# EugenHotaj/pytorch-generative

Measured on NVIDIA H100. Metric: images/sec training step (ImageGPT CIFAR-10 32x32), higher is better.
Workload: dtype bf16

## Files before the change

### pytorch_generative_b200/csrc/pg_gemm.cu

```cuda
#include <stdlib.h>
#include <string.h>

#include "../../include/pg_b200.h"
#include "pg_common.cuh"

namespace {

constexpr int BM = 128;
constexpr int BK = 64;
constexpr int A_STAGE_BYTES = BM * BK * 2;
constexpr int SMEM_LIMIT = 232448;

constexpr int MAX_CONV_TAPS = 225;
struct ConvGeom {
  int mode, H, W, C, T;
  int cslabs;
  int nbpt;
  int8_t dy[MAX_CONV_TAPS], dx[MAX_CONV_TAPS];
};

struct GemmParams {
  ConvGeom conv;
  int M, N, K;
  int num_m_blk, num_n_blk;
  int k_iters;
  int k_per_split;
  int splits;
  int stages;
  int epi_tma, epi_nbuf, epi_buf_bytes, epi_in_bytes;
  int off_old, off_res0, off_res1, off_aux, off_f32, off_pre, off_bf16;
  int epi_smem;
  int store_deriv;
  int res_bf16;
  float* a_rowsum;
  float* split_part;
  float* rowsum_part;
  pg_gemm_epilogue epi;
};

struct EpiMaps {
  CUtensorMap res0, res1, aux, out_f32, out_pre, out_bf16;
  CUtensorMap bias;
};

template <bool BWD, int ACT, int N>
__device__ __forceinline__ void act_as(float (&x)[N]) {
#pragma unroll
  for (int i = 0; i < N; ++i) x[i] = BWD ? pg_act_bwd(ACT, x[i]) : pg_act_fwd(ACT, x[i]);
}
template <bool BWD, int N>
__device__ __forceinline__ void act_n(int act, float (&x)[N]) {
  switch (act) {
    case PG_ACT_RELU: act_as<BWD, PG_ACT_RELU>(x); break;
    case PG_ACT_GELU: act_as<BWD, PG_ACT_GELU>(x); break;
    case PG_ACT_ELU: act_as<BWD, PG_ACT_ELU>(x); break;
    case PG_ACT_TANH: act_as<BWD, PG_ACT_TANH>(x); break;
    case PG_ACT_GIVEN: act_as<BWD, PG_ACT_GIVEN>(x); break;
    case PG_ACT_RELU_OUT: act_as<BWD, PG_ACT_RELU_OUT>(x); break;
    case PG_ACT_ELU_OUT: act_as<BWD, PG_ACT_ELU_OUT>(x); break;
    default: act_as<BWD, PG_ACT_NONE>(x); break;
  }
}

__device__ __forceinline__ void epilogue_row32(const GemmParams& p, int row, int col0, int ncols, bool first_split,
                                               const uint32_t (&acc)[32], float* out_f32, int64_t ld_out_f32,
                                               bool accumulate) {
  const pg_gemm_epilogue& e = p.epi;
  float v[32];
#pragma unroll
  for (int i = 0; i < 32; ++i) v[i] = __uint_as_float(acc[i]) * e.alpha;

  if (first_split && e.bias) {
    for (int i = 0; i < ncols; ++i) v[i] += __ldg(e.bias + col0 + i);
  }
  if (e.dact != PG_ACT_NONE) {
    const bf16* aux = reinterpret_cast<const bf16*>(e.aux) + (size_t)row * e.ld_aux + col0;
    for (int i = 0; i < ncols; ++i) v[i] *= pg_act_bwd(e.dact, __bfloat162float(aux[i]));
  }
#pragma unroll
  for (int which = 0; which < 2; ++which) {
    const float* rp = which == 0 ? e.res0 : e.res1;
    if (first_split && rp && p.res_bf16) {
      const bf16* r = reinterpret_cast<const bf16*>(rp) + (size_t)row * e.ld_res + col0;
      for (int i = 0; i < ncols; ++i) v[i] += __bfloat162float(r[i]);
    } else if (first_split && rp) {
      const float* r = rp + (size_t)row * e.ld_res + col0;
      for (int i = 0; i < ncols; ++i) v[i] += r[i];
    }
  }
  if (out_f32) {
    float* o = out_f32 + (size_t)row * ld_out_f32 + col0;
    if (accumulate) {
      for (int i = 0; i < ncols; ++i) o[i] += v[i];
    } else {
      for (int i = 0; i < ncols; ++i) o[i] = v[i];
    }
  }
  if (e.out_pre) {
    bf16* o = reinterpret_cast<bf16*>(e.out_pre) + (size_t)row * e.ld_out_pre + col0;
    float d[32];
#pragma unroll
    for (int i = 0; i < 32; ++i) d[i] = v[i];
    if (p.store_deriv) act_n<true>(e.act, d);
    for (int i = 0; i < ncols; ++i) o[i] = __float2bfloat16(d[i]);
  }
  if (e.out_bf16) {
    bf16* o = reinterpret_cast<bf16*>(e.out_bf16) + (size_t)row * e.ld_out_bf16 + col0;
    if (e.act != PG_ACT_NONE) act_n<false>(e.act, v);
    for (int i = 0; i < ncols; ++i) o[i] = __float2bfloat16(v[i]);
  }
}

constexpr int GEMM_THREADS = 384;
constexpr int XP_LD = 68;
constexpr int XP_BYTES = 64 * XP_LD * 4;
constexpr int MAX_STAGES = 8;
constexpr int MAX_EPI_BUFS = 4;
constexpr int EPI_F32_BYTES = 16 * 32 * 4;
constexpr int EPI_BF16_BYTES = 16 * 32 * 2;
constexpr int EPI_BIAS_BYTES = 128 * 4;
constexpr int PRODUCER_REGS = 56;
constexpr int CONSUMER_REGS = 224;
constexpr uint32_t XPOSE_BAR = 1;
constexpr uint32_t ROWSUM_BAR = 3;
constexpr uint32_t MMA_TURN_BAR = 4;

struct WorkItem {
  int m_blk, n_blk, ks, k0, k1;
};
__device__ __forceinline__ WorkItem work_item(const GemmParams& p, int tile) {
  WorkItem w;
  w.n_blk = tile % p.num_n_blk;
  const int rest = tile / p.num_n_blk;
  w.m_blk = rest % p.num_m_blk;
  w.ks = rest / p.num_m_blk;
  w.k0 = w.ks * p.k_per_split;
  w.k1 = min(w.k0 + p.k_per_split, p.k_iters);
  return w;
}

template <int BN, bool A_MN, bool B_MN>
__device__ __forceinline__ void consumer_mainloop(uint8_t* smem, uint64_t* full_bar, uint64_t* empty_bar, int stages,
                                                  const WorkItem& w, int& s, uint32_t& ph, float (&acc)[2][BN / 2],
                                                  int turn_bar) {
  constexpr int STAGE_BYTES = A_STAGE_BYTES + BN * BK * 2;
  const int lane = threadIdx.x & 31;
  int prev = -1;
  for (int kit = w.k0; kit < w.k1; ++kit) {
    mbar_wait(&full_bar[s], ph);
    const uint32_t a_addr = smem_u32(smem + s * STAGE_BYTES);
    const uint32_t b_addr = smem_u32(smem + s * STAGE_BYTES) + A_STAGE_BYTES;
    const uint64_t b_base = B_MN ? wgmma_desc_sw128(b_addr, BK * 128, 1024) : wgmma_desc_sw128(b_addr, 16, 1024);
    wgmma_fence();
#pragma unroll
    for (int kk = 0; kk < BK / 16; ++kk) {
#pragma unroll
      for (int sl = 0; sl < 2; ++sl) {
        const uint32_t sa = a_addr + sl * (64 * 128);
        const uint64_t a_base = A_MN ? wgmma_desc_sw128(sa, BK * 128, 1024) : wgmma_desc_sw128(sa, 16, 1024);
        Wgmma<BN>::template ss<A_MN ? 1 : 0, B_MN ? 1 : 0>(acc[sl], a_base + (uint64_t)(A_MN ? kk * 128 : kk * 2),
                                                         b_base + (uint64_t)(B_MN ? kk * 128 : kk * 2),
                                                         (kit > w.k0 || kk > 0) ? 1u : 0u);
      }
    }
    wgmma_commit();
    wgmma_wait<1>();
    if (prev >= 0) {
      __syncwarp();
      if (lane == 0) mbar_arrive(&empty_bar[prev]);
    }
    prev = s;
    if (++s == stages) { s = 0; ph ^= 1; }
  }
  if (turn_bar >= 0) named_bar_arrive((uint32_t)turn_bar, 256);
  wgmma_wait<0>();
#pragma unroll
  for (int sl = 0; sl < 2; ++sl) wgmma_hold(acc[sl]);
  if (prev >= 0) {
    __syncwarp();
    if (lane == 0) mbar_arrive(&empty_bar[prev]);
  }
}

template <int BN>
__device__ __forceinline__ void consumer_epilogue(const GemmParams& p, const WorkItem& w, const float (&acc)[2][BN / 2],
                                                  float* xp, uint32_t xbar) {
  constexpr int CSTEPS = (BN + 63) / 64;
  const int t = threadIdx.x & 127, lane = threadIdx.x & 31, wi = (threadIdx.x >> 5) & 3;
  const int r = t & 63, half = t >> 6;
#pragma unroll 1
  for (int step = 0; step < 2 * CSTEPS; ++step) {
    const int sl = step / CSTEPS, c0 = (step - sl * CSTEPS) * 64;
    const int row = w.m_blk * BM + sl * 64 + r;
    named_bar_sync(xbar, 128);
#pragma unroll
    for (int q = 0; q < 2; ++q) {
#pragma unroll
      for (int j = 0; j < BN / 8; ++j) {
        if (q == sl && j * 8 >= c0 && j * 8 < c0 + 64) {
          const int col = j * 8 - c0 + 2 * (lane & 3), fr = wi * 16 + (lane >> 2);
          *reinterpret_cast<float2*>(xp + fr * XP_LD + col) = make_float2(acc[q][4 * j], acc[q][4 * j + 1]);
          *reinterpret_cast<float2*>(xp + (fr + 8) * XP_LD + col) = make_float2(acc[q][4 * j + 2], acc[q][4 * j + 3]);
        }
      }
    }
    named_bar_sync(xbar, 128);
    const int col0 = w.n_blk * BN + c0 + half * 32;
    if (c0 + half * 32 < BN && row < p.M && col0 < p.N) {
      uint32_t v[32];
#pragma unroll
      for (int u = 0; u < 8; ++u) {
        const float4 x = *reinterpret_cast<const float4*>(xp + r * XP_LD + half * 32 + 4 * u);
        v[4 * u] = __float_as_uint(x.x); v[4 * u + 1] = __float_as_uint(x.y);
        v[4 * u + 2] = __float_as_uint(x.z); v[4 * u + 3] = __float_as_uint(x.w);
      }
      const bool split = p.split_part != nullptr;
      epilogue_row32(p, row, col0, min(32, p.N - col0), w.ks == 0, v,
                     split ? p.split_part + (size_t)w.ks * p.M * p.N : p.epi.out_f32,
                     split ? (int64_t)p.N : p.epi.ld_out_f32, !split && p.epi.accumulate);
    }
  }
}

struct EpiRing {
  uint8_t* buf;
  float* bias;
  uint64_t* in_bar;
  uint64_t* bias_bar;
};
__device__ __forceinline__ EpiRing epi_ring(const GemmParams& p, uint8_t* epi, int cw) {
  const int wq = cw * 4 + ((threadIdx.x >> 5) & 3);
  EpiRing r;
  r.buf = epi + wq * p.epi_nbuf * p.epi_buf_bytes;
  r.bias = reinterpret_cast<float*>(epi + 8 * p.epi_nbuf * p.epi_buf_bytes + cw * EPI_BIAS_BYTES);
  r.in_bar = reinterpret_cast<uint64_t*>(epi + p.epi_smem) + 2 * MAX_STAGES + wq * MAX_EPI_BUFS;
  r.bias_bar = reinterpret_cast<uint64_t*>(epi + p.epi_smem) + 2 * MAX_STAGES + 8 * MAX_EPI_BUFS + cw;
  return r;
}

constexpr int EK_GENERIC = 0;
constexpr int EK_BIAS = 1, EK_GIVEN = 2, EK_RES0 = 4, EK_RES1 = 8, EK_F32 = 16, EK_BF16 = 32, EK_GELU2 = 64;
constexpr int EK_PLAIN = EK_BF16;
constexpr int EK_BIAS_BF16 = EK_BIAS | EK_BF16;
constexpr int EK_BIAS_GELU2 = EK_BIAS | EK_GELU2;
constexpr int EK_GIVEN_BF16 = EK_GIVEN | EK_BF16;
constexpr int EK_BIAS_RES_F32 = EK_BIAS | EK_RES0 | EK_F32;
constexpr int EK_BIAS_RES2_F32 = EK_BIAS | EK_RES0 | EK_RES1 | EK_F32;

__device__ __forceinline__ bool subtile_live(const GemmParams& p, int row, int col) { return row < p.M && col < p.N; }

template <int BN>
__device__ __forceinline__ void epi_load(const GemmParams& p, const EpiMaps& tm, const WorkItem& w, const EpiRing& r,
                                         int g0, int j) {
  constexpr int CG = BN / 32;
  const int wi = (threadIdx.x >> 5) & 3;
  const int b = (g0 + j) % p.epi_nbuf;
  uint8_t* buf = r.buf + b * p.epi_buf_bytes;
  const int col = w.n_blk * BN + (j % CG) * 32, row = w.m_blk * BM + (j / CG) * 64 + wi * 16;
  if (!subtile_live(p, row, col)) {
    mbar_arrive(&r.in_bar[b]);
    return;
  }
  mbar_arrive_expect_tx(&r.in_bar[b], (uint32_t)p.epi_in_bytes);
  if (p.off_old >= 0) tma_load_3d(buf + p.off_old, &tm.out_f32, &r.in_bar[b], col, row, 0);
  if (p.off_res0 >= 0) tma_load_2d(buf + p.off_res0, &tm.res0, &r.in_bar[b], col, row);
  if (p.off_res1 >= 0) tma_load_2d(buf + p.off_res1, &tm.res1, &r.in_bar[b], col, row);
  if (p.off_aux >= 0) tma_load_2d(buf + p.off_aux, &tm.aux, &r.in_bar[b], col, row);
}

template <int BN>
__device__ __forceinline__ void epi_prologue(const GemmParams& p, const EpiMaps& tm, const WorkItem& w, const EpiRing& r,
                                             int item) {
  if ((threadIdx.x & 31) != 0 || !p.epi_in_bytes) return;
  bulk_wait_group_read<1>();
  for (int j = 0; j < p.epi_nbuf - 1 && j < 2 * (BN / 32); ++j) epi_load<BN>(p, tm, w, r, item * 2 * (BN / 32), j);
}

template <int BN>
__device__ __forceinline__ void epi_bias(const GemmParams& p, const EpiMaps& tm, const WorkItem& w, const EpiRing& r) {
  if ((threadIdx.x & 127) != 0 || !p.epi.bias) return;
  mbar_arrive_expect_tx(r.bias_bar, BN * 4);
  tma_load_1d(r.bias, &tm.bias, r.bias_bar, w.n_blk * BN);
}

template <int BN, int EK, bool ACT>
__device__ __forceinline__ void consumer_epilogue_tma(const GemmParams& p, const EpiMaps& tm, const WorkItem& w,
                                                      const float (&acc)[2][BN / 2], const EpiRing& r, int item) {
  constexpr int CG = BN / 32, NSUB = 2 * CG;
  constexpr bool G = EK == EK_GENERIC;
  const pg_gemm_epilogue& e = p.epi;
  const int lane = threadIdx.x & 31, wi = (threadIdx.x >> 5) & 3;
  const int nb = p.epi_nbuf, g0 = item * NSUB;
  const bool bias = G ? e.bias != nullptr : (EK & EK_BIAS) != 0;
  const bool has_in = G ? p.epi_in_bytes != 0 : (EK & (EK_GIVEN | EK_RES0)) != 0;
  const bool f32_out = G ? p.off_f32 >= 0 : (EK & EK_F32) != 0;
  const bool bf16_out = G ? p.off_bf16 >= 0 : (EK & (EK_BF16 | EK_GELU2)) != 0;
  const bool pre_out = G ? p.off_pre >= 0 : (EK & EK_GELU2) != 0;
  if (bias) mbar_wait(r.bias_bar, (uint32_t)item & 1u);
  const uint32_t rb = lane >> 2;
  const uint32_t f32_base = rb * 128 + ((((uint32_t)lane >> 1) & 1u) ^ (rb & 7u)) * 16 + (lane & 1) * 8;
  const uint32_t bf_base = rb * 64 + ((rb >> 1) & 3u) * 16 + (lane & 3) * 4;
  auto f32_at = [&](int jj, int hi) { return (f32_base ^ (uint32_t)(jj << 5)) + hi * 1024; };
  auto bf_at = [&](int jj, int hi) { return (bf_base ^ (uint32_t)(jj << 4)) + hi * 512; };
  int b = g0 % nb;
  uint32_t par = (uint32_t)(g0 / nb) & 1u;
#pragma unroll(G ? 1 : NSUB)
  for (int i = 0; i < NSUB; ++i) {
    const int sl = i / CG, cg = i - sl * CG;
    uint8_t* buf = r.buf + b * p.epi_buf_bytes;
    float v[16];
#pragma unroll
    for (int q = 0; q < 2; ++q)
#pragma unroll
      for (int c = 0; c < CG; ++c)
        if (q == sl && c == cg) {
#pragma unroll
          for (int k = 0; k < 16; ++k) v[k] = acc[q][c * 16 + k];
        }
    if (has_in) mbar_wait(&r.in_bar[b], par);
    if (G) {
#pragma unroll
      for (int k = 0; k < 16; ++k) v[k] *= e.alpha;
    }
    if (bias) {
#pragma unroll
      for (int jj = 0; jj < 4; ++jj) {
        const float2 bb = *reinterpret_cast<const float2*>(r.bias + cg * 32 + jj * 8 + 2 * (lane & 3));
        v[4 * jj] += bb.x; v[4 * jj + 1] += bb.y; v[4 * jj + 2] += bb.x; v[4 * jj + 3] += bb.y;
      }
    }
    if ((G && ACT && e.dact != PG_ACT_NONE) || (EK & EK_GIVEN)) {
#pragma unroll
      for (int h = 0; h < 2; ++h) {
        float g[8];
#pragma unroll
        for (int jj = 0; jj < 2; ++jj)
#pragma unroll
          for (int hi = 0; hi < 2; ++hi) {
            const float2 f =
                unpack_bf16x2(*reinterpret_cast<const uint32_t*>(buf + p.off_aux + bf_at(2 * h + jj, hi)));
            g[4 * jj + 2 * hi] = f.x;
            g[4 * jj + 2 * hi + 1] = f.y;
          }
        if (G) act_n<true>(e.dact, g);
#pragma unroll
        for (int k = 0; k < 8; ++k) v[8 * h + k] *= g[k];
      }
    }
#pragma unroll
    for (int which = 0; which < 2; ++which) {
      const bool res = G ? (which == 0 ? p.off_res0 : p.off_res1) >= 0 : (EK & (which == 0 ? EK_RES0 : EK_RES1)) != 0;
      if (!res) continue;
      const int off = which == 0 ? p.off_res0 : p.off_res1;
      const bool res_bf16 = G && p.res_bf16;
#pragma unroll
      for (int jj = 0; jj < 4; ++jj)
#pragma unroll
        for (int hi = 0; hi < 2; ++hi) {
          const float2 f = res_bf16 ? unpack_bf16x2(*reinterpret_cast<const uint32_t*>(buf + off + bf_at(jj, hi)))
                                    : *reinterpret_cast<const float2*>(buf + off + f32_at(jj, hi));
          v[4 * jj + 2 * hi] += f.x;
          v[4 * jj + 2 * hi + 1] += f.y;
        }
    }
    __syncwarp();
    if (f32_out) {
      const bool old = G && p.off_old >= 0;
#pragma unroll
      for (int jj = 0; jj < 4; ++jj)
#pragma unroll
        for (int hi = 0; hi < 2; ++hi) {
          float2* o = reinterpret_cast<float2*>(buf + p.off_f32 + f32_at(jj, hi));
          float2 f = make_float2(v[4 * jj + 2 * hi], v[4 * jj + 2 * hi + 1]);
          if (old) {
            const float2 ov = *o;
            f = make_float2(ov.x + f.x, ov.y + f.y);
          }
          *o = f;
        }
    }
    bool v_act = false;
    if (pre_out) {
      float d[16];
      if ((EK & EK_GELU2) || (G && ACT && p.store_deriv && e.act == PG_ACT_GELU)) {
#pragma unroll
        for (int k = 0; k < 16; ++k) pg_gelu_both(v[k], v[k], d[k]);
        v_act = true;
      } else {
#pragma unroll
        for (int k = 0; k < 16; ++k) d[k] = v[k];
        if (G && ACT && p.store_deriv) act_n<true>(e.act, d);
      }
#pragma unroll
      for (int jj = 0; jj < 4; ++jj)
#pragma unroll
        for (int hi = 0; hi < 2; ++hi)
          *reinterpret_cast<uint32_t*>(buf + p.off_pre + bf_at(jj, hi)) =
              pack_bf16x2(d[4 * jj + 2 * hi], d[4 * jj + 2 * hi + 1]);
    }
    if (bf16_out) {
      if (G && ACT && !v_act && e.act != PG_ACT_NONE) act_n<false>(e.act, v);
#pragma unroll
      for (int jj = 0; jj < 4; ++jj)
#pragma unroll
        for (int hi = 0; hi < 2; ++hi)
          *reinterpret_cast<uint32_t*>(buf + p.off_bf16 + bf_at(jj, hi)) =
              pack_bf16x2(v[4 * jj + 2 * hi], v[4 * jj + 2 * hi + 1]);
    }
    fence_proxy_async_smem();
    __syncwarp();
    if (lane == 0) {
      const int col = w.n_blk * BN + cg * 32, row = w.m_blk * BM + sl * 64 + wi * 16;
      if (subtile_live(p, row, col)) {
        if (f32_out) tma_store_3d(&tm.out_f32, buf + p.off_f32, col, row, w.ks);
        if (pre_out) tma_store_2d(&tm.out_pre, buf + p.off_pre, col, row);
        if (bf16_out) tma_store_2d(&tm.out_bf16, buf + p.off_bf16, col, row);
      }
      bulk_commit_group();
      if (has_in) {
        bulk_wait_group_read<1>();
        if (i + nb - 1 < NSUB) epi_load<BN>(p, tm, w, r, g0, i + nb - 1);
      } else if (nb == 4) {
        bulk_wait_group_read<3>();
      } else if (nb == 3) {
        bulk_wait_group_read<2>();
      } else {
        bulk_wait_group_read<1>();
      }
    }
    if (++b == nb) { b = 0; par ^= 1u; }
  }
}

template <int BN, bool A_MN, bool B_MN, int EK>
__global__ void __launch_bounds__(GEMM_THREADS, 1)
gemm_wgmma_kernel(const __grid_constant__ CUtensorMap tmA, const __grid_constant__ CUtensorMap tmB,
                  const __grid_constant__ EpiMaps tmE, const GemmParams p) {
  constexpr int STAGE_BYTES = A_STAGE_BYTES + BN * BK * 2;
  extern __shared__ uint8_t smem_raw[];
  uint8_t* smem = smem_raw + ((1024u - (smem_u32(smem_raw) & 1023u)) & 1023u);
  const int STAGES = p.stages;
  uint8_t* const epi = smem + STAGES * STAGE_BYTES;
  uint64_t* full_bar = reinterpret_cast<uint64_t*>(epi + p.epi_smem);
  uint64_t* empty_bar = full_bar + MAX_STAGES;
  uint64_t* in_bar = empty_bar + MAX_STAGES;
  uint64_t* bias_bar = in_bar + 8 * MAX_EPI_BUFS;
  float* rowsum_xch = reinterpret_cast<float*>(bias_bar + 2);

  const int warp = threadIdx.x >> 5;
  const int lane = threadIdx.x & 31;
  const bool rowsum = A_MN && p.a_rowsum != nullptr;
  const int num_tiles = p.num_m_blk * p.num_n_blk * p.splits;
  if (threadIdx.x == 0) {
    tma_prefetch_desc(&tmA);
    tma_prefetch_desc(&tmB);
    for (int i = 0; i < STAGES; ++i) {
      mbar_init(&full_bar[i], 1);
      mbar_init(&empty_bar[i], rowsum ? 6 : 4);
    }
    for (int i = 0; i < 8 * MAX_EPI_BUFS + 2; ++i) mbar_init(&in_bar[i], 1);
    fence_barrier_init();
    fence_proxy_async_smem();
  }
  __syncthreads();

  if (warp < 4) {
    setmaxnreg_dec<PRODUCER_REGS>();
    if (warp == 0) {
      int s = 0;
      uint32_t ph = 0;
      for (int tile = blockIdx.x; tile < num_tiles; tile += gridDim.x) {
        const WorkItem w = work_item(p, tile);
        const int m_blk = w.m_blk, n_blk = w.n_blk;
        for (int kit = w.k0; kit < w.k1; ++kit) {
          mbar_wait(&empty_bar[s], ph ^ 1);
          uint8_t* sA = smem + s * STAGE_BYTES;
          uint8_t* sB = sA + A_STAGE_BYTES;
          mbar_arrive_expect_tx_w(&full_bar[s], STAGE_BYTES);
          if (p.conv.mode != 0) {
            const int hw = p.conv.H * p.conv.W;
            if (p.conv.mode == 1) {
              const int t = kit / p.conv.cslabs, cs = kit - t * p.conv.cslabs;
              const int row0 = m_blk * BM, n = row0 / hw, h0 = (row0 - n * hw) / p.conv.W;
              tma_load_4d_w(sA, &tmA, &full_bar[s], cs * 64, p.conv.dx[t], h0 + p.conv.dy[t], n);
              if (!B_MN) {
                tma_load_2d_w(sB, &tmB, &full_bar[s], kit * BK, n_blk * BN);
              } else {
#pragma unroll
                for (int j = 0; j < BN / 64; ++j)
                  tma_load_2d_w(sB + j * (BK * 128), &tmB, &full_bar[s], t * p.N + n_blk * BN + j * 64, cs * 64);
              }
            } else {
              const int t = n_blk / p.conv.nbpt, nb = n_blk - t * p.conv.nbpt;
              const int pix0 = kit * BK, n = pix0 / hw, h0 = (pix0 - n * hw) / p.conv.W;
#pragma unroll
              for (int j = 0; j < BM / 64; ++j)
                tma_load_2d_w(sA + j * (BK * 128), &tmA, &full_bar[s], m_blk * BM + j * 64, kit * BK);
#pragma unroll
              for (int j = 0; j < BN / 64; ++j)
                tma_load_4d_w(sB + j * (BK * 128), &tmB, &full_bar[s], nb * BN + j * 64, p.conv.dx[t], h0 + p.conv.dy[t], n);
            }
          } else {
            if (!A_MN) {
              tma_load_2d_w(sA, &tmA, &full_bar[s], kit * BK, m_blk * BM);
            } else {
#pragma unroll
              for (int j = 0; j < BM / 64; ++j)
                tma_load_2d_w(sA + j * (BK * 128), &tmA, &full_bar[s], m_blk * BM + j * 64, kit * BK);
            }
            if (!B_MN) {
              tma_load_2d_w(sB, &tmB, &full_bar[s], kit * BK, n_blk * BN);
            } else {
#pragma unroll
              for (int j = 0; j < BN / 64; ++j)
                tma_load_2d_w(sB + j * (BK * 128), &tmB, &full_bar[s], n_blk * BN + j * 64, kit * BK);
            }
          }
          if (++s == STAGES) { s = 0; ph ^= 1; }
        }
      }
    } else if (A_MN && (warp == 2 || warp == 3)) {
      if (rowsum) {
        const int t = (warp - 2) * 32 + lane;
        const int c = t & 15, g = t >> 4;
        const uint32_t atom = (uint32_t)(c >> 3) * (BK * 128), cc = (uint32_t)(c & 7);
        int s = 0;
        uint32_t ph = 0;
        for (int tile = blockIdx.x; tile < num_tiles; tile += gridDim.x) {
          const WorkItem w = work_item(p, tile);
          const bool mine = (w.n_blk == 0);
          float acc[8];
#pragma unroll
          for (int q = 0; q < 8; ++q) acc[q] = 0.f;
          for (int kit = w.k0; kit < w.k1; ++kit) {
            mbar_wait(&full_bar[s], ph);
            if (mine) {
              const uint8_t* sA = smem + s * STAGE_BYTES + atom;
#pragma unroll
              for (int i = 0; i < BK / 4; ++i) {
                const uint32_t k = (uint32_t)(g + 4 * i);
                const uint4 v = *reinterpret_cast<const uint4*>(sA + k * 128 + ((cc ^ (k & 7u)) << 4));
                const uint32_t ww[4] = {v.x, v.y, v.z, v.w};
#pragma unroll
                for (int j = 0; j < 4; ++j) {
                  const float2 f = unpack_bf16x2(ww[j]);
                  acc[2 * j] += f.x;
                  acc[2 * j + 1] += f.y;
                }
              }
            }
            __syncwarp();
            if (lane == 0) mbar_arrive(&empty_bar[s]);
            if (++s == STAGES) { s = 0; ph ^= 1; }
          }
          if (mine) {
#pragma unroll
            for (int q = 0; q < 8; ++q) acc[q] += __shfl_xor_sync(0xffffffffu, acc[q], 16);
            named_bar_sync(ROWSUM_BAR, 64);
            if (warp == 3 && lane < 16) {
#pragma unroll
              for (int q = 0; q < 8; ++q) rowsum_xch[lane * 8 + q] = acc[q];
            }
            named_bar_sync(ROWSUM_BAR, 64);
            if (warp == 2 && lane < 16) {
#pragma unroll
              for (int q = 0; q < 8; ++q) acc[q] += rowsum_xch[lane * 8 + q];
              const int m0 = w.m_blk * BM + c * 8;
#pragma unroll
              for (int q = 0; q < 8; ++q)
                if (m0 + q < p.M) {
                  if (p.rowsum_part) p.rowsum_part[(size_t)w.ks * p.M + m0 + q] = acc[q];
                  else p.a_rowsum[m0 + q] += acc[q];
                }
            }
          }
        }
      }
    }
  } else {
    setmaxnreg_inc<CONSUMER_REGS>();
    const int cw = (warp - 4) >> 2;
    float* const xp = reinterpret_cast<float*>(epi) + cw * 64 * XP_LD;
    float acc[2][BN / 2];
    int s = 0;
    uint32_t ph = 0;
    int i = 0;
    for (int tile = blockIdx.x; tile < num_tiles; tile += gridDim.x, ++i) {
      const WorkItem w = work_item(p, tile);
      if ((i & 1) != cw) {
        const int pos = s + (w.k1 - w.k0);
        ph ^= (uint32_t)((pos / STAGES) & 1);
        s = pos % STAGES;
        continue;
      }
      const bool has_next = tile + (int)gridDim.x < num_tiles;
      if (p.epi_tma) epi_prologue<BN>(p, tmE, w, epi_ring(p, epi, cw), i >> 1);
      if (i > 0) named_bar_sync(MMA_TURN_BAR + cw, 256);
      if (p.epi_tma) epi_bias<BN>(p, tmE, w, epi_ring(p, epi, cw));
      consumer_mainloop<BN, A_MN, B_MN>(smem, full_bar, empty_bar, STAGES, w, s, ph, acc,
                                        has_next ? (int)(MMA_TURN_BAR + (cw ^ 1)) : -1);
      if constexpr (BN <= 64) {
        if (!p.epi_tma) consumer_epilogue<BN>(p, w, acc, xp, XPOSE_BAR + cw);
      }
      if (p.epi_tma) {
        const EpiRing r = epi_ring(p, epi, cw);
        if constexpr (EK != EK_GENERIC)
          consumer_epilogue_tma<BN, EK, false>(p, tmE, w, acc, r, i >> 1);
        else if (p.epi.act == PG_ACT_NONE && p.epi.dact == PG_ACT_NONE && !p.store_deriv)
          consumer_epilogue_tma<BN, EK, false>(p, tmE, w, acc, r, i >> 1);
        else
          consumer_epilogue_tma<BN, EK, true>(p, tmE, w, acc, r, i >> 1);
      }
    }
    if (lane == 0) bulk_wait_group_all();
  }
}

__global__ void gemm_simt_kernel(const bf16* __restrict__ A, int a_mn, int64_t lda, const bf16* __restrict__ B,
                                 int b_mn, int64_t ldb, const GemmParams p) {
  const int nseg = (p.N + 31) / 32;
  const long long idx = (long long)blockIdx.x * blockDim.x + threadIdx.x;
  if (idx >= (long long)p.M * nseg) return;
  const int row = (int)(idx / nseg);
  const int col0 = (int)(idx % nseg) * 32;
  const int ncols = min(32, p.N - col0);
  float acc[32];
#pragma unroll
  for (int i = 0; i < 32; ++i) acc[i] = 0.f;
  for (int k = 0; k < p.K; ++k) {
    const float a = __bfloat162float(a_mn ? A[(size_t)k * lda + row] : A[(size_t)row * lda + k]);
    for (int i = 0; i < ncols; ++i) {
      const int n = col0 + i;
      const float b = __bfloat162float(b_mn ? B[(size_t)k * ldb + n] : B[(size_t)n * ldb + k]);
      acc[i] = fmaf(a, b, acc[i]);
    }
  }
  uint32_t accu[32];
#pragma unroll
  for (int i = 0; i < 32; ++i) accu[i] = __float_as_uint(acc[i]);
  epilogue_row32(p, row, col0, ncols, true, accu, p.epi.out_f32, p.epi.ld_out_f32, p.epi.accumulate != 0);
}

__global__ void __launch_bounds__(256)
gemm_skinny_kernel(const bf16* __restrict__ A, int64_t lda, const bf16* __restrict__ B, int64_t ldb, const GemmParams p) {
  extern __shared__ uint4 sA4[];
  const int lane = threadIdx.x & 31, warp = threadIdx.x >> 5;
  const int K8 = p.K / 8;
  for (int i = threadIdx.x; i < p.M * K8; i += blockDim.x)
    sA4[i] = *reinterpret_cast<const uint4*>(A + (size_t)(i / K8) * lda + (i % K8) * 8);
  __syncthreads();
  const int n = blockIdx.x * 8 + warp;
  if (n >= p.N) return;
  float acc[32];
#pragma unroll
  for (int m = 0; m < 32; ++m) acc[m] = 0.f;
  const uint4* wrow = reinterpret_cast<const uint4*>(B + (size_t)n * ldb);
  for (int k8 = lane; k8 < K8; k8 += 32) {
    const uint4 wv = __ldg(wrow + k8);
    const uint32_t ww[4] = {wv.x, wv.y, wv.z, wv.w};
    float wf[8];
#pragma unroll
    for (int j = 0; j < 4; ++j) {
      const float2 f = unpack_bf16x2(ww[j]);
      wf[2 * j] = f.x;
      wf[2 * j + 1] = f.y;
    }
#pragma unroll
    for (int m = 0; m < 32; ++m) {
      if (m < p.M) {
        const uint4 av = sA4[m * K8 + k8];
        const uint32_t aw[4] = {av.x, av.y, av.z, av.w};
#pragma unroll
        for (int j = 0; j < 4; ++j) {
          const float2 f = unpack_bf16x2(aw[j]);
          acc[m] = fmaf(f.x, wf[2 * j], fmaf(f.y, wf[2 * j + 1], acc[m]));
        }
      }
    }
  }
  float mine = 0.f;
#pragma unroll
  for (int m = 0; m < 32; ++m) {
    if (m < p.M) {
      const float v = warp_sum(acc[m]);
      if (lane == m) mine = v;
    }
  }
  if (lane < p.M) {
    const pg_gemm_epilogue& e = p.epi;
    const int m = lane;
    float t = mine * e.alpha;
    if (e.bias) t += e.bias[n];
    if (p.res_bf16) {
      if (e.res0) t += __bfloat162float(reinterpret_cast<const bf16*>(e.res0)[(size_t)m * e.ld_res + n]);
      if (e.res1) t += __bfloat162float(reinterpret_cast<const bf16*>(e.res1)[(size_t)m * e.ld_res + n]);
    } else {
      if (e.res0) t += e.res0[(size_t)m * e.ld_res + n];
      if (e.res1) t += e.res1[(size_t)m * e.ld_res + n];
    }
    if (e.out_f32) e.out_f32[(size_t)m * e.ld_out_f32 + n] = t;
    if (e.out_pre)
      reinterpret_cast<bf16*>(e.out_pre)[(size_t)m * e.ld_out_pre + n] =
          __float2bfloat16(p.store_deriv ? pg_act_bwd(e.act, t) : t);
    if (e.out_bf16) reinterpret_cast<bf16*>(e.out_bf16)[(size_t)m * e.ld_out_bf16 + n] = __float2bfloat16(pg_act_fwd(e.act, t));
  }
}

int epi_kind(const GemmParams& p) {
  const pg_gemm_epilogue& e = p.epi;
  if (!p.epi_tma || e.alpha != 1.f || p.res_bf16 || p.off_old >= 0 || p.splits > 1) return EK_GENERIC;
  const bool bias = e.bias != nullptr, f32 = e.out_f32 != nullptr, bf = e.out_bf16 != nullptr;
  const bool pre = e.out_pre != nullptr, res0 = e.res0 != nullptr, res1 = e.res1 != nullptr;
  const bool no_act = e.act == PG_ACT_NONE && !p.store_deriv;
  if (bf && !f32 && !pre && !res0 && !res1 && no_act && e.dact == PG_ACT_NONE) return bias ? EK_BIAS_BF16 : EK_PLAIN;
  if (bf && !f32 && !pre && !res0 && !res1 && no_act && e.dact == PG_ACT_GIVEN && !bias) return EK_GIVEN_BF16;
  if (bf && pre && !f32 && !res0 && !res1 && bias && e.act == PG_ACT_GELU && p.store_deriv && e.dact == PG_ACT_NONE)
    return EK_BIAS_GELU2;
  if (f32 && !bf && !pre && res0 && bias && no_act && e.dact == PG_ACT_NONE)
    return res1 ? EK_BIAS_RES2_F32 : EK_BIAS_RES_F32;
  return EK_GENERIC;
}

template <int BN, bool A_MN, bool B_MN>
int launch_tc(const void* A, int64_t lda, const void* B, int64_t ldb, GemmParams& p, cudaStream_t stream) {
  CUtensorMap tmA, tmB;
  const ConvGeom& cg = p.conv;
  auto conv_map = [&](CUtensorMap* out, const void* base, int64_t ld, int pixels_per_box) {
    const int64_t n_img = (cg.mode == 1 ? (int64_t)p.M : (int64_t)p.K) / ((int64_t)cg.H * cg.W);
    uint64_t dims[4] = {(uint64_t)cg.C, (uint64_t)cg.W, (uint64_t)cg.H, (uint64_t)n_img};
    uint64_t strides[3] = {(uint64_t)ld * 2, (uint64_t)cg.W * ld * 2, (uint64_t)cg.H * cg.W * ld * 2};
    uint32_t box[4] = {64, (uint32_t)cg.W, (uint32_t)(pixels_per_box / cg.W), 1};
    return pg_make_tmap_nd_bf16(out, base, 4, dims, strides, box, 1);
  };
  if (cg.mode == 1) {
    if (conv_map(&tmA, A, lda, BM)) return 1;
  } else if (!A_MN) {
    if (pg_make_tmap_2d_bf16(&tmA, A, p.M, p.K, lda, BM, BK)) return 1;
  } else {
    if (pg_make_tmap_2d_bf16(&tmA, A, p.K, p.M, lda, BK, 64)) return 1;
  }
  if (cg.mode == 2) {
    PG_REQUIRE(B_MN && cg.C % BN == 0, "pg_gemm_bf16_conv(wgrad): channels (%d) must be a multiple of the N tile (%d)", cg.C, BN);
    p.conv.nbpt = cg.C / BN;
    if (conv_map(&tmB, B, ldb, BK)) return 1;
  } else if (!B_MN) {
    if (pg_make_tmap_2d_bf16(&tmB, B, p.N, p.K, ldb, BN, BK)) return 1;
  } else if (cg.mode == 1) {
    if (pg_make_tmap_2d_bf16(&tmB, B, cg.C, (uint64_t)cg.T * p.N, ldb, BK, 64)) return 1;
  } else {
    if (pg_make_tmap_2d_bf16(&tmB, B, p.K, p.N, ldb, BK, 64)) return 1;
  }
  EpiMaps tmE;
  memset(&tmE, 0, sizeof(tmE));
  if (p.epi_tma) {
    const pg_gemm_epilogue& e = p.epi;
    auto f32_map = [&](CUtensorMap* out, const void* base, int64_t ld) {
      return pg_make_tmap_2d(out, base, 4, p.M, p.N, ld, 16, 32, 128);
    };
    auto bf16_map = [&](CUtensorMap* out, const void* base, int64_t ld) {
      return pg_make_tmap_2d(out, base, 2, p.M, p.N, ld, 16, 32, 64);
    };
    if (e.res0 && (p.res_bf16 ? bf16_map(&tmE.res0, e.res0, e.ld_res) : f32_map(&tmE.res0, e.res0, e.ld_res))) return 1;
    if (e.res1 && (p.res_bf16 ? bf16_map(&tmE.res1, e.res1, e.ld_res) : f32_map(&tmE.res1, e.res1, e.ld_res))) return 1;
    if (p.off_aux >= 0 && bf16_map(&tmE.aux, e.aux, e.ld_aux)) return 1;
    if (e.out_pre && bf16_map(&tmE.out_pre, e.out_pre, e.ld_out_pre)) return 1;
    if (e.out_bf16 && bf16_map(&tmE.out_bf16, e.out_bf16, e.ld_out_bf16)) return 1;
    if (e.out_f32) {
      const float* base = p.split_part ? p.split_part : e.out_f32;
      const uint64_t ld = p.split_part ? (uint64_t)p.N : (uint64_t)e.ld_out_f32;
      const uint64_t dims[3] = {(uint64_t)p.N, (uint64_t)p.M, (uint64_t)p.splits};
      const uint64_t strides[2] = {ld * 4, ld * 4 * (uint64_t)p.M};
      const uint32_t box[3] = {32, 16, 1};
      if (pg_make_tmap_nd(&tmE.out_f32, base, 4, 3, dims, strides, box, 128)) return 1;
    }
    if (e.bias) {
      const uint64_t dims[1] = {(uint64_t)p.N};
      const uint32_t box[1] = {(uint32_t)BN};
      if (pg_make_tmap_nd(&tmE.bias, e.bias, 4, 1, dims, nullptr, box, 0)) return 1;
    }
  }
  constexpr int STAGE_BYTES = A_STAGE_BYTES + BN * BK * 2;
  const int fixed = 1024  + (2 * MAX_STAGES + 8 * MAX_EPI_BUFS + 2) * 8  +
                    16 * 8 * 4 ;
  const int avail = SMEM_LIMIT - fixed;
  if (p.epi_tma) {
    const int bufs_room = (avail - 2 * EPI_BIAS_BYTES - 4 * STAGE_BYTES) / (8 * p.epi_buf_bytes);
    p.epi_nbuf = min(min(MAX_EPI_BUFS, 2 * (BN / 32)), max(2, bufs_room));
    p.epi_smem = 8 * p.epi_nbuf * p.epi_buf_bytes + 2 * EPI_BIAS_BYTES;
  } else {
    p.epi_nbuf = 0;
    p.epi_smem = 2 * XP_BYTES;
  }
  int stages = (avail - p.epi_smem) / STAGE_BYTES;
  if (stages > MAX_STAGES) stages = MAX_STAGES;
  if (stages > p.k_iters + 1) stages = p.k_iters + 1 > 2 ? p.k_iters + 1 : 2;
  PG_REQUIRE(stages >= 2, "pg_gemm_bf16: %d bytes of epilogue staging leave no room for two pipeline stages",
             p.epi_smem);
  p.stages = stages;
  const int smem_bytes = stages * STAGE_BYTES + p.epi_smem + fixed;
  auto kern = gemm_wgmma_kernel<BN, A_MN, B_MN, EK_GENERIC>;
  if constexpr (BN == 128 && !A_MN) {
    switch (epi_kind(p)) {
      case EK_PLAIN: kern = gemm_wgmma_kernel<BN, A_MN, B_MN, EK_PLAIN>; break;
      case EK_BIAS_BF16: kern = gemm_wgmma_kernel<BN, A_MN, B_MN, EK_BIAS_BF16>; break;
      case EK_BIAS_GELU2: kern = gemm_wgmma_kernel<BN, A_MN, B_MN, EK_BIAS_GELU2>; break;
      case EK_GIVEN_BF16: kern = gemm_wgmma_kernel<BN, A_MN, B_MN, EK_GIVEN_BF16>; break;
      case EK_BIAS_RES_F32: kern = gemm_wgmma_kernel<BN, A_MN, B_MN, EK_BIAS_RES_F32>; break;
      case EK_BIAS_RES2_F32: kern = gemm_wgmma_kernel<BN, A_MN, B_MN, EK_BIAS_RES2_F32>; break;
      default: break;
    }
  }
  PG_CUDA(cudaFuncSetAttribute(kern, cudaFuncAttributeMaxDynamicSharedMemorySize, smem_bytes));
  const int num_tiles = p.num_m_blk * p.num_n_blk * p.splits;
  const int grid = min(num_tiles, pg_num_sms());
  kern<<<grid, GEMM_THREADS, smem_bytes, stream>>>(tmA, tmB, tmE, p);
  if (pg_check_launch("pg_gemm_bf16(wgmma)")) return 1;
  if (p.split_part &&
      pg_sum_partials(p.split_part, p.splits, (long long)p.M * p.N, p.M, p.N, p.epi.ld_out_f32, p.epi.out_f32, stream))
    return 1;
  if (p.rowsum_part && pg_sum_partials(p.rowsum_part, p.splits, p.M, 1, p.M, p.M, p.a_rowsum, stream)) return 1;
  return 0;
}

template <bool A_MN, bool B_MN>
int dispatch_bn(const void* A, int64_t lda, const void* B, int64_t ldb, GemmParams& p, cudaStream_t stream) {
  int bn;
  if (p.N > 64) bn = 128;
  else if (p.N > 32) bn = 64;
  else bn = 32;
  if (!p.epi_tma && bn > 64) bn = 64;
  if (B_MN && bn < 64) bn = 64;
  if (p.conv.mode == 2) bn = (p.conv.C % 128 == 0 && p.epi_tma) ? 128 : 64;
  p.num_n_blk = (p.N + bn - 1) / bn;
  switch (bn) {
    case 128: return launch_tc<128, A_MN, B_MN>(A, lda, B, ldb, p, stream);
    case 64: return launch_tc<64, A_MN, B_MN>(A, lda, B, ldb, p, stream);
    default: return launch_tc<32, A_MN, B_MN>(A, lda, B, ldb, p, stream);
  }
}

}

static int gemm_entry(const void* A, int a_mn_major, int64_t lda, const void* B, int b_mn_major, int64_t ldb, int M, int N,
                      int K, int split_k, const pg_gemm_epilogue* epi, int impl, const ConvGeom* conv, void* stream_) {
  cudaStream_t stream = reinterpret_cast<cudaStream_t>(stream_);
  PG_REQUIRE(A && B && epi, "pg_gemm_bf16: null operand");
  PG_REQUIRE(M > 0 && N > 0 && K > 0, "pg_gemm_bf16: empty problem M=%d N=%d K=%d", M, N, K);
  PG_REQUIRE(lda % 8 == 0 && ldb % 8 == 0, "pg_gemm_bf16: pitches must be multiples of 8 elements (lda=%lld ldb=%lld)",
             (long long)lda, (long long)ldb);
  PG_REQUIRE(epi->out_bf16 || epi->out_pre || epi->out_f32, "pg_gemm_bf16: no output requested");
  PG_REQUIRE(epi->dact == PG_ACT_NONE || epi->aux, "pg_gemm_bf16: dact needs aux");
  if (split_k < 1) split_k = 1;
  if (split_k > 1)
    PG_REQUIRE(epi->accumulate && epi->out_f32 && !epi->out_bf16 && !epi->out_pre && epi->dact == PG_ACT_NONE &&
                   !epi->bias && !epi->res0 && !epi->res1,
               "pg_gemm_bf16: split_k > 1 requires accumulate=1 into out_f32 only (no bias / residuals)");
  GemmParams p;
  memset(&p, 0, sizeof(p));
  if (conv) p.conv = *conv;
  p.M = M; p.N = N; p.K = K;
  p.num_m_blk = (M + BM - 1) / BM;
  p.num_n_blk = 0;
  p.k_iters = (K + BK - 1) / BK;
  if (split_k > p.k_iters) split_k = p.k_iters;
  p.k_per_split = (p.k_iters + split_k - 1) / split_k;
  p.splits = (p.k_iters + p.k_per_split - 1) / p.k_per_split;
  p.epi = *epi;
  p.store_deriv = (epi->act & PG_ACT_STORE_DERIV) ? 1 : 0;
  p.res_bf16 = (epi->act & PG_ACT_RES_BF16) ? 1 : 0;
  p.epi.act = epi->act & 0xff;
  p.a_rowsum = epi->bias_grad;
  PG_REQUIRE(!epi->bias_grad || (a_mn_major && impl == 0),
             "pg_gemm_bf16: bias_grad rides on the weight-gradient GEMM (a_mn_major = 1, impl 0)");
  PG_REQUIRE(!p.store_deriv || epi->out_pre, "pg_gemm_bf16: PG_ACT_STORE_DERIV needs out_pre");
  auto al16 = [](const void* q) { return (reinterpret_cast<uintptr_t>(q) & 15) == 0; };
  bool vec_ok = true;
  if (epi->bias && !al16(epi->bias)) vec_ok = false;
  const bool aux = epi->dact != PG_ACT_NONE;
  if (aux && (!al16(epi->aux) || epi->ld_aux % 8)) vec_ok = false;
  const int res_mult = p.res_bf16 ? 8 : 4;
  if (epi->res0 && (!al16(epi->res0) || epi->ld_res % res_mult)) vec_ok = false;
  if (epi->res1 && (!al16(epi->res1) || epi->ld_res % res_mult)) vec_ok = false;
  if (epi->out_f32 && (!al16(epi->out_f32) || epi->ld_out_f32 % 4)) vec_ok = false;
  if (epi->out_pre && (!al16(epi->out_pre) || epi->ld_out_pre % 8)) vec_ok = false;
  if (epi->out_bf16 && (!al16(epi->out_bf16) || epi->ld_out_bf16 % 8)) vec_ok = false;
  if (N % 8) vec_ok = false;
  p.epi_tma = vec_ok ? 1 : 0;
  p.off_old = p.off_res0 = p.off_res1 = p.off_aux = p.off_f32 = p.off_pre = p.off_bf16 = -1;
  if (p.epi_tma) {
    const int res_bytes = p.res_bf16 ? EPI_BF16_BYTES : EPI_F32_BYTES;
    int in = 0, out = 0;
    if (epi->accumulate && epi->out_f32 && p.splits == 1) { p.off_old = in; in += EPI_F32_BYTES; }
    if (epi->res0) { p.off_res0 = in; in += res_bytes; }
    if (epi->res1) { p.off_res1 = in; in += res_bytes; }
    if (aux) { p.off_aux = in; in += EPI_BF16_BYTES; }
    if (epi->out_f32) { p.off_f32 = out; out += EPI_F32_BYTES; }
    if (epi->out_pre) { p.off_pre = out; out += EPI_BF16_BYTES; }
    if (epi->out_bf16) { p.off_bf16 = out; out += EPI_BF16_BYTES; }
    p.epi_in_bytes = in;
    p.epi_buf_bytes = in > out ? in : out;
  }

  if (impl == 1) {
    p.splits = 1;
    p.k_per_split = p.k_iters;
    const int nseg = (N + 31) / 32;
    const long long total = (long long)M * nseg;
    const int threads = 128;
    const long long blocks = (total + threads - 1) / threads;
    gemm_simt_kernel<<<(unsigned)blocks, threads, 0, stream>>>(reinterpret_cast<const bf16*>(A), a_mn_major, lda,
                                                                 reinterpret_cast<const bf16*>(B), b_mn_major, ldb, p);
    return pg_check_launch("pg_gemm_bf16(simt)");
  }
  if (impl == 2) {
    PG_REQUIRE(!a_mn_major && !b_mn_major && M <= 32 && !epi->accumulate && epi->dact == PG_ACT_NONE && K % 8 == 0 &&
                   (reinterpret_cast<uintptr_t>(A) & 15) == 0 && (reinterpret_cast<uintptr_t>(B) & 15) == 0 &&
                   (size_t)M * K * 2 <= 160 * 1024,
               "pg_gemm_bf16(skinny): needs a K-major forward GEMM with M <= 32 rows (M=%d K=%d)", M, K);
    const size_t smem = (size_t)M * K * 2;
    PG_CUDA(cudaFuncSetAttribute(gemm_skinny_kernel, cudaFuncAttributeMaxDynamicSharedMemorySize, 160 * 1024));
    gemm_skinny_kernel<<<(N + 7) / 8, 256, smem, stream>>>(reinterpret_cast<const bf16*>(A), lda,
                                                           reinterpret_cast<const bf16*>(B), ldb, p);
    return pg_check_launch("pg_gemm_bf16(skinny)");
  }
  if (p.splits > 1) {
    const size_t mn = (size_t)M * N, rows = p.a_rowsum ? (size_t)M : 0;
    float* part = nullptr;
    if (pg_scratch((size_t)p.splits * (mn + rows) * sizeof(float), stream, &part)) return 1;
    p.split_part = part;
    if (p.a_rowsum) p.rowsum_part = part + (size_t)p.splits * mn;
  }
  if (!a_mn_major && !b_mn_major) return dispatch_bn<false, false>(A, lda, B, ldb, p, stream);
  if (!a_mn_major && b_mn_major) return dispatch_bn<false, true>(A, lda, B, ldb, p, stream);
  if (a_mn_major && b_mn_major) return dispatch_bn<true, true>(A, lda, B, ldb, p, stream);
  return dispatch_bn<true, false>(A, lda, B, ldb, p, stream);
}

extern "C" int pg_gemm_bf16(const void* A, int a_mn_major, int64_t lda, const void* B, int b_mn_major, int64_t ldb,
                            int M, int N, int K, int split_k, const pg_gemm_epilogue* epi, int impl, void* stream_) {
  return gemm_entry(A, a_mn_major, lda, B, b_mn_major, ldb, M, N, K, split_k, epi, impl, nullptr, stream_);
}

extern "C" int pg_gemm_bf16_conv_taps(const void* A, int64_t lda, const void* B, int64_t ldb, int M, int N, int K,
                                      int split_k, const pg_gemm_epilogue* epi, int mode, int n_img, int H, int W, int C,
                                      int n_taps, const int* dy, const int* dx, void* stream_) {
  PG_REQUIRE(mode >= PG_CONV_FWD && mode <= PG_CONV_WGRAD, "pg_gemm_bf16_conv: mode %d", mode);
  PG_REQUIRE(n_taps >= 1 && n_taps <= MAX_CONV_TAPS, "pg_gemm_bf16_conv: 1..%d taps (got %d)", MAX_CONV_TAPS, n_taps);
  PG_REQUIRE(dy && dx, "pg_gemm_bf16_conv: null tap offsets");
  PG_REQUIRE(C % 64 == 0 && W >= 1 && W <= 64 && 64 % W == 0 && ((int64_t)H * W) % 128 == 0,
             "pg_gemm_bf16_conv: needs C %% 64 == 0, W | 64 and H*W %% 128 == 0 (C=%d H=%d W=%d); use pg_tap_gather otherwise",
             C, H, W);
  const int64_t P = (int64_t)n_img * H * W;
  ConvGeom cg;
  memset(&cg, 0, sizeof(cg));
  cg.H = H; cg.W = W; cg.C = C; cg.T = n_taps;
  cg.cslabs = C / 64;
  for (int t = 0; t < n_taps; ++t) {
    PG_REQUIRE(dy[t] >= -64 && dy[t] <= 64 && dx[t] >= -64 && dx[t] <= 64, "pg_gemm_bf16_conv: tap offset out of range");
    cg.dy[t] = (int8_t)dy[t];
    cg.dx[t] = (int8_t)dx[t];
  }
  if (mode == PG_CONV_WGRAD) {
    PG_REQUIRE(K == P && N == n_taps * C, "pg_gemm_bf16_conv(wgrad): K must be N*H*W and N = taps * C");
    cg.mode = 2;
    return gemm_entry(A, 1, lda, B, 1, ldb, M, N, K, split_k, epi, 0, &cg, stream_);
  }
  PG_REQUIRE(M == P && K == n_taps * C, "pg_gemm_bf16_conv: M must be N*H*W and K = taps * C");
  cg.mode = 1;
  return gemm_entry(A, 0, lda, B, mode == PG_CONV_DGRAD ? 1 : 0, ldb, M, N, K, split_k, epi, 0, &cg, stream_);
}

extern "C" int pg_gemm_bf16_conv(const void* A, int64_t lda, const void* B, int64_t ldb, int M, int N, int K, int split_k,
                                 const pg_gemm_epilogue* epi, const pg_conv_geom* g, void* stream_) {
  PG_REQUIRE(g, "pg_gemm_bf16_conv: null geometry");
  PG_REQUIRE(g->n_taps >= 1 && g->n_taps <= 32, "pg_gemm_bf16_conv: 1..32 taps in a pg_conv_geom (got %d)", g->n_taps);
  return pg_gemm_bf16_conv_taps(A, lda, B, ldb, M, N, K, split_k, epi, g->mode, g->N, g->H, g->W, g->C, g->n_taps, g->dy,
                                g->dx, stream_);
}
```

Before: 536.9.

## Offload rowsum to idle consumer warpgroup when CTA has a single tile

When a CTA processes only one tile, the second consumer warpgroup would otherwise sit idle. It now computes the A row-sum with 128 threads using vectorized shared loads, instead of producer warps 2-3 doing it, and the empty-barrier arrival count is adjusted to match. The existing multi-tile rowsum path also batches four ld.shared.v4 loads before accumulating, to raise memory-level parallelism. This risks extra barrier complexity and shared-memory scratch aliasing with the epilogue buffers.

```diff
diff --git a/pytorch_generative_b200/csrc/pg_gemm.cu b/pytorch_generative_b200/csrc/pg_gemm.cu
--- a/pytorch_generative_b200/csrc/pg_gemm.cu
+++ b/pytorch_generative_b200/csrc/pg_gemm.cu
@@ -125,6 +125,17 @@
 constexpr uint32_t ROWSUM_BAR = 3;
 constexpr uint32_t MMA_TURN_BAR = 4;
 
+__device__ __forceinline__ uint2 ld_shared_v2(uint32_t addr) {
+  uint2 v;
+  asm volatile("ld.shared.v2.u32 {%0, %1}, [%2];" : "=r"(v.x), "=r"(v.y) : "r"(addr));
+  return v;
+}
+__device__ __forceinline__ uint4 ld_shared_v4(uint32_t addr) {
+  uint4 v;
+  asm volatile("ld.shared.v4.u32 {%0, %1, %2, %3}, [%4];" : "=r"(v.x), "=r"(v.y), "=r"(v.z), "=r"(v.w) : "r"(addr));
+  return v;
+}
+
 struct WorkItem {
   int m_blk, n_blk, ks, k0, k1;
 };
@@ -137,6 +148,48 @@
   w.k0 = w.ks * p.k_per_split;
   w.k1 = min(w.k0 + p.k_per_split, p.k_iters);
   return w;
+}
+
+__device__ __forceinline__ bool rowsum_writer(const GemmParams&, const WorkItem& w) { return w.n_blk == 0; }
+
+template <int BN>
+__device__ __forceinline__ void rowsum_warpgroup(const GemmParams& p, uint8_t* smem, uint64_t* full_bar,
+                                                 uint64_t* empty_bar, int stages, const WorkItem& w, float* xch) {
+  constexpr int STAGE_BYTES = A_STAGE_BYTES + BN * BK * 2;
+  const int t = threadIdx.x & 127, g = t >> 5, h = t & 31, lane = t & 31;
+  const uint32_t cc = (uint32_t)((h & 15) >> 1);
+  const uint32_t base = (uint32_t)(h >> 4) * (BK * 128) + (uint32_t)g * 128 + (uint32_t)(h & 1) * 8;
+  const uint32_t off0 = base + ((cc ^ (uint32_t)g) << 4), off1 = base + ((cc ^ (uint32_t)g ^ 4u) << 4);
+  float acc[4] = {0.f, 0.f, 0.f, 0.f};
+  int s = 0;
+  uint32_t ph = 0;
+  for (int kit = w.k0; kit < w.k1; ++kit) {
+    mbar_wait(&full_bar[s], ph);
+    const uint32_t sA = smem_u32(smem + s * STAGE_BYTES);
+    uint2 v[BK / 4];
+#pragma unroll
+    for (int i = 0; i < BK / 4; ++i) v[i] = ld_shared_v2(sA + ((i & 1) ? off1 : off0) + (uint32_t)i * 512);
+#pragma unroll
+    for (int i = 0; i < BK / 4; ++i) {
+      const float2 f0 = unpack_bf16x2(v[i].x), f1 = unpack_bf16x2(v[i].y);
+      acc[0] += f0.x;
+      acc[1] += f0.y;
+      acc[2] += f1.x;
+      acc[3] += f1.y;
+    }
+    __syncwarp();
+    if (lane == 0) mbar_arrive(&empty_bar[s]);
+    if (++s == stages) { s = 0; ph ^= 1; }
+  }
+#pragma unroll
+  for (int q = 0; q < 4; ++q) xch[g * 128 + h * 4 + q] = acc[q];
+  named_bar_sync(XPOSE_BAR + 1, 128);
+  const int m = w.m_blk * BM + t;
+  if (m < p.M) {
+    const float v = (xch[t] + xch[128 + t]) + (xch[256 + t] + xch[384 + t]);
+    if (p.rowsum_part) p.rowsum_part[(size_t)w.ks * p.M + m] = v;
+    else p.a_rowsum[m] += v;
+  }
 }
 
 template <int BN, bool A_MN, bool B_MN>
@@ -451,12 +504,14 @@
   const int lane = threadIdx.x & 31;
   const bool rowsum = A_MN && p.a_rowsum != nullptr;
   const int num_tiles = p.num_m_blk * p.num_n_blk * p.splits;
+  const bool single = blockIdx.x + (int)gridDim.x >= num_tiles;
+  const bool wg_rowsum = rowsum && single && rowsum_writer(p, work_item(p, blockIdx.x));
   if (threadIdx.x == 0) {
     tma_prefetch_desc(&tmA);
     tma_prefetch_desc(&tmB);
     for (int i = 0; i < STAGES; ++i) {
       mbar_init(&full_bar[i], 1);
-      mbar_init(&empty_bar[i], rowsum ? 6 : 4);
+      mbar_init(&empty_bar[i], 4 + (!rowsum ? 0 : !single ? 2 : wg_rowsum ? 4 : 0));
     }
     for (int i = 0; i < 8 * MAX_EPI_BUFS + 2; ++i) mbar_init(&in_bar[i], 1);
     fence_barrier_init();
@@ -520,7 +575,7 @@
         }
       }
     } else if (A_MN && (warp == 2 || warp == 3)) {
-      if (rowsum) {
+      if (rowsum && !single) {
         const int t = (warp - 2) * 32 + lane;
         const int c = t & 15, g = t >> 4;
         const uint32_t atom = (uint32_t)(c >> 3) * (BK * 128), cc = (uint32_t)(c & 7);
@@ -528,24 +583,29 @@
         uint32_t ph = 0;
         for (int tile = blockIdx.x; tile < num_tiles; tile += gridDim.x) {
           const WorkItem w = work_item(p, tile);
-          const bool mine = (w.n_blk == 0);
+          const bool mine = rowsum_writer(p, w);
           float acc[8];
 #pragma unroll
           for (int q = 0; q < 8; ++q) acc[q] = 0.f;
           for (int kit = w.k0; kit < w.k1; ++kit) {
             mbar_wait(&full_bar[s], ph);
             if (mine) {
-              const uint8_t* sA = smem + s * STAGE_BYTES + atom;
-#pragma unroll
-              for (int i = 0; i < BK / 4; ++i) {
-                const uint32_t k = (uint32_t)(g + 4 * i);
-                const uint4 v = *reinterpret_cast<const uint4*>(sA + k * 128 + ((cc ^ (k & 7u)) << 4));
-                const uint32_t ww[4] = {v.x, v.y, v.z, v.w};
-#pragma unroll
-                for (int j = 0; j < 4; ++j) {
-                  const float2 f = unpack_bf16x2(ww[j]);
-                  acc[2 * j] += f.x;
-                  acc[2 * j + 1] += f.y;
+              const uint32_t sA = smem_u32(smem + s * STAGE_BYTES + atom) + (uint32_t)g * 128;
+              const uint32_t a0 = sA + ((cc ^ (uint32_t)g) << 4), a1 = sA + ((cc ^ (uint32_t)g ^ 4u) << 4);
+#pragma unroll
+              for (int h = 0; h < BK / 16; ++h) {
+                uint4 v[4];
+#pragma unroll
+                for (int i = 0; i < 4; ++i) v[i] = ld_shared_v4(((i & 1) ? a1 : a0) + (uint32_t)(4 * h + i) * 512);
+#pragma unroll
+                for (int i = 0; i < 4; ++i) {
+                  const uint32_t ww[4] = {v[i].x, v[i].y, v[i].z, v[i].w};
+#pragma unroll
+                  for (int j = 0; j < 4; ++j) {
+                    const float2 f = unpack_bf16x2(ww[j]);
+                    acc[2 * j] += f.x;
+                    acc[2 * j + 1] += f.y;
+                  }
                 }
               }
             }
@@ -581,6 +641,11 @@
     setmaxnreg_inc<CONSUMER_REGS>();
     const int cw = (warp - 4) >> 2;
     float* const xp = reinterpret_cast<float*>(epi) + cw * 64 * XP_LD;
+    if (cw == 1 && wg_rowsum) {
+      float* xch = p.epi_tma ? reinterpret_cast<float*>(epi + 4 * p.epi_nbuf * p.epi_buf_bytes) : xp;
+      rowsum_warpgroup<BN>(p, smem, full_bar, empty_bar, STAGES, work_item(p, blockIdx.x), xch);
+      return;
+    }
     float acc[2][BN / 2];
     int s = 0;
     uint32_t ph = 0;
```

Measured after the change: 552.2 (median of 6 runs). 1.03x the previous value.
